# Hippogriff/prifit

Hardware: AMD Instinct MI355X
Metric: shapes/sec (fwd+bwd) B=24x2048 pts, PointNet++-MSG+ellipsoid fit (higher is better)
Workload: dtype f32; 1 GPU; configs[2]: PointNet++-MSG + mean-shift(10 it, <=25 clusters) + ellipsoid fit + convex loss, B=24x2048 per GPU, fwd+bwd+Adam; global_batch=24, points=2048, parallelism=dp1, cloud=blobs, embedding=clustered, backbone_grad_param=sa1.conv_blocks.0.0.weight, launch=eager

## Files before the change

include/prifit_hip.h:

```cpp
#ifndef PRIFIT_HIP_H
#define PRIFIT_HIP_H

#include <stdint.h>

#ifdef __cplusplus
extern "C" {
#endif

#define PRIFIT_OK 0
#define PRIFIT_EINVAL (-1)
#define PRIFIT_ELAUNCH (-2)

#define PRIFIT_ABI_VERSION 700
int prifit_version(const char **arch);


int prifit_fps(const float *xyz, int B, int N, int npoint, const int64_t *start_idx,
               int64_t *out_idx, float *new_xyz, void *stream);

int prifit_ball_query(const float *xyz, const float *new_xyz, int B, int N, int S, int R,
                      const float *radius2, const int *nsample, void *const *out, int idx64,
                      void *stream);

int prifit_three_nn(const float *xyz1, const float *xyz2, int B, int N, int S, int32_t *idx,
                    float *dist, float *weight, void *stream);

int prifit_square_distance(const float *src, const float *dst, int B, int S, int N, float *out,
                           void *stream);


int prifit_group_gather(const float *feat, const float *xyz, const float *new_xyz,
                        const int32_t *idx, int B, int N, int S, int K, int C, int order,
                        int ld_out, float *out, void *stream);

int prifit_group_scatter_add(const float *gout, int ld_gout, int col0, const int32_t *idx, int B,
                             int N, int S, int K, int C, float *dfeat, void *stream);
// ... 12 lines not shown

int prifit_three_interpolate_bwd(const float *gout, int ld_gout, int col0, const int32_t *idx,
                                 const float *weight, int B, int N, int S, int C, float *dpoints2,
                                 void *stream);
int prifit_fp_rows(const float *points2, const int32_t *idx, const float *weight, const float *points1, int B, int N, int S, int D2,
                   int D1, int kp, float *out, void *stream);


#define PRIFIT_GEMM_NT 0
#define PRIFIT_GEMM_NN 1
#define PRIFIT_GEMM_TN 2
#define PRIFIT_EPI_NONE 0
#define PRIFIT_EPI_CHORD 1
#define PRIFIT_EPI_MSKERNEL 2
#define PRIFIT_EPI_MSBWD 3

int prifit_gemm_f32(int layout, int M, int N, int K, const float *A, long long lda, long long strideA,
                    const float *B, long long ldb, long long strideB, float *C, long long ldc,
                    long long strideC, int batch, int splitk, const float *a_scale,
                    const float *a_shift, const float *b_scale, const float *b_shift,
                    const float *bias, long long bias_batch_stride, float *col_stats, int epilogue,
                    const float *epi_batch_scalar, const float *epi_aux, long long ld_aux,
                    long long stride_aux, const float *epi_row_add, float *a_rowsum, int accumulate, void *stream);

int prifit_chord_sym_f32(const float *A, long long lda, long long strideA, float *C, long long ldc, long long strideC,
                         int n, int K, int batch, unsigned long long *owner_key, void *stream);
int prifit_chord_sym_mask(const float *A, long long lda, long long strideA, const float *thr, uint32_t *mask, int n, int K, int batch,
                          unsigned long long *owner_key, void *stream);
int prifit_gram_sym_f32(const float *A, long long lda, long long strideA, float *C, long long ldc, long long strideC, int n, int K,
                        int batch, void *stream);

int prifit_gemm_pool_f32(int M, int N, int K, const float *A, long long lda, const float *W, long long ldb, float *Y,
                         long long ldc, const float *a_scale, const float *a_shift, const float *bias, float *col_stats,
                         float *cand, void *stream);
int prifit_gemm_pool_supported(int M, int N, int K);

int prifit_gemm_stream_f32(int layout, int M, int N, int K, const float *A, long long lda, const float *B,
                           long long ldb, float *C, long long ldc, const float *a_scale, const float *a_shift,
                           const float *bias, float *col_stats, void *stream);
int prifit_gemm_stream_supported(int layout, int M, int N, int K);
int prifit_gemm_stream_slabs(int M, int K);

int prifit_gemm_dual_nn_f32(int M, int N, int K1, int K2, const float *A1, const float *A2, long long lda,
                            long long strideA, const float *B1, const float *B2, long long ldb, long long strideB,
                            float *C, long long ldc, long long strideC, int batch, int splitk, int accumulate,
                            void *stream);
// ... 386 lines not shown
```

prifit_amd/_lib.py:

```python
import ctypes
import os
import re

import torch

_HERE = os.path.dirname(os.path.abspath(__file__))
LIB_PATH = os.environ.get("PRIFIT_LIB") or os.path.join(_HERE, "lib", "libprifit_hip.so")
HEADER_PATH = os.path.join(os.path.dirname(_HERE), "include", "prifit_hip.h")

_P = ctypes.c_void_p
_I = ctypes.c_int
_F = ctypes.c_float
_D = ctypes.c_double
_LL = ctypes.c_longlong

_dll = None


def declared_symbols(header_path=HEADER_PATH):
    return sorted(_declared(header_path))


def _declared(header_path=HEADER_PATH):
    with open(header_path) as f:
        text = f.read()
    return {name: ret for ret, name in re.findall(r"^\s*(int|long long)\s+(prifit_\w+)\s*\(", text, flags=re.M)}


def _ctype_of(param):
    p = param.strip()
    if p in ("void", ""):
        return None
    if "*" in p or "[" in p:
        return ctypes.c_void_p
    if re.search(r"\blong\s+long\b", p):
        return ctypes.c_ulonglong if "unsigned" in p else ctypes.c_longlong
    if re.search(r"\bdouble\b", p):
        return ctypes.c_double
    if re.search(r"\bfloat\b", p):
# ... 98 lines not shown
```

prifit_amd/csrc/gemm.hip:

```cpp
#include <stdlib.h>

#include <type_traits>

#include "common.h"

typedef float f32x16 __attribute__((ext_vector_type(16)));

enum { LAY_NT = 0, LAY_NN = 1, LAY_TN = 2 };
enum { EPI_NONE = 0, EPI_CHORD = 1, EPI_MSKERNEL = 2, EPI_MSBWD = 3, EPI_BNRED = 4 };

struct GemmArgs {
    const float *A, *B;
    float *C;
    int M, N, K;
    long long lda, ldb, ldc;
    long long sA, sB, sC;
    int batch, splitk;
    const float *a_scale, *a_shift;
    const float *b_scale, *b_shift;
    const float *bias;
    long long bias_stride;
    float *stats;
    int epi;
    const float *epi_batch_scalar;
    const float *aux;
    const float *row_add;
    float *a_rowsum;
    long long ldaux, sAux;
    const float *red_scale, *red_shift, *red_mean, *red_invstd;
    long long dA2, dB2;
    int kswitch;
    int accumulate;
    int vecA, vecB;
    int ntiles;
    float *cand;
};

#ifndef GEMM_W8
#define GEMM_W8 6
#endif
constexpr int BK = 32;
constexpr int PAD = 4;

__device__ __forceinline__ float4 ld4(const float *p) { return *reinterpret_cast<const float4 *>(p); }

template <int ROWS, bool KC, bool VEC, bool AFF, int NTH>
struct TileLoader {
    static constexpr int NV = ROWS * BK / 4 / NTH;
    static_assert(NV * NTH * 4 == ROWS * BK, "tile must divide evenly over the threads");
    float4 v[NV];
    const float *ptr[NV];
    int klo[NV];
    int c0[NV];
    unsigned okmask[NV];
    long long step;
    int K, R, cclamp;

    __device__ __forceinline__ void init(const float *__restrict__ base, long long ld, int r0, int R_, int K_)
    {
// ... 292 lines not shown
            fa[(gk + 1) & 1] = read_frag<RA, AKC>(As, arow, gk + 1, lh);
#pragma unroll
            for (int b = 0; b < TN; ++b)
                if (b < nbv) fb[(gk + 1) & 1][b] = read_frag<RB, BKC>(Bs, bcol + 32 * b, gk + 1, lh);
        }
        __builtin_amdgcn_sched_barrier(0);
        const float4 a = fa[gk & 1];
#pragma unroll
        for (int b = 0; b < TN; ++b) {
            if (b >= nbv) continue;
            const float4 w = fb[gk & 1][b];
            acc[b] = __builtin_amdgcn_mfma_f32_32x32x2f32(a.x, w.x, acc[b], 0, 0, 0);
            acc[b] = __builtin_amdgcn_mfma_f32_32x32x2f32(a.y, w.y, acc[b], 0, 0, 0);
            acc[b] = __builtin_amdgcn_mfma_f32_32x32x2f32(a.z, w.z, acc[b], 0, 0, 0);
            acc[b] = __builtin_amdgcn_mfma_f32_32x32x2f32(a.w, w.w, acc[b], 0, 0, 0);
        }
        __builtin_amdgcn_sched_barrier(0);
    }
}

template <bool C, class A, class B> struct pick { typedef A type; };
template <class A, class B> struct pick<false, A, B> { typedef B type; };

template <int BM, int BN, int WM, int WN, int LAY, bool VA, bool VB, bool FA, bool FB, bool EX = false>
__global__ __launch_bounds__((BM / WM) * (BN / WN) * 64, ((BM / WM) * (BN / WN) == 8 ? GEMM_W8 : 4)) void gemm_kernel(const GemmArgs g)
{
    constexpr int NTH = (BM / WM) * (BN / WN) * 64;
    constexpr bool A_KC = (LAY != LAY_TN);
    constexpr bool B_KC = (LAY == LAY_NT);
    constexpr int TM = WM / 32, TN = WN / 32;
    constexpr int WAVES_N = BN / WN;
    static_assert(NTH == 256 || NTH == 512, "4 or 8 waves per block");
    constexpr int SZA = A_KC ? BM * (BK + PAD) : BK * (BM + PAD);
    constexpr int SZB = B_KC ? BN * (BK + PAD) : BK * (BN + PAD);
    __shared__ __attribute__((aligned(16))) float lds[2 * (SZA + SZB)];

    const int tilesN = (g.N + BN - 1) / BN;
    const int nwg = gridDim.x;
    int L;
    {
        const int bid = blockIdx.x, xcd = bid & 7, pos = bid >> 3, q = nwg >> 3, r = nwg & 7;
        L = (xcd < r ? xcd * (q + 1) : r * (q + 1) + (xcd - r) * q) + pos;
    }
    const int tile_m = L / tilesN, tile_n = L - tile_m * tilesN;
    const int m0 = tile_m * BM, n0 = tile_n * BN;
    const int z = blockIdx.z / g.splitk, ks = blockIdx.z - z * g.splitk;

    const float *A = g.A + (long long)z * g.sA;
    const float *B = g.B + (long long)z * g.sB;
    float *C = g.C + (long long)z * g.sC;

    const int ktiles = (g.K + BK - 1) / BK;
    const int per = (ktiles + g.splitk - 1) / g.splitk;
    const int kt0 = ks * per, kt1 = min(ktiles, kt0 + per);

    const int wave = threadIdx.x >> 6, lane = threadIdx.x & 63;
    const int li = lane & 31, lh = lane >> 5;
    const int wm0 = (wave / WAVES_N) * WM, wn0 = (wave % WAVES_N) * WN;

    f32x16 acc[TM][TN];
#pragma unroll
    for (int a = 0; a < TM; ++a)
#pragma unroll
        for (int b = 0; b < TN; ++b)
#pragma unroll
            for (int r = 0; r < 16; ++r) acc[a][b][r] = 0.f;

    typename pick<EX, BufLoader<BM, A_KC, FA, NTH>, TileLoader<BM, A_KC, VA, FA, NTH>>::type la;
    typename pick<EX, BufLoader<BN, B_KC, FB, NTH>, TileLoader<BN, B_KC, VB, FB, NTH>>::type lb;
// ... 174 lines not shown
        }
    }
    if (g.stats) {
        __syncthreads();
        float *red = lds;
#pragma unroll
        for (int b = 0; b < TN; ++b) {
            float s = csum[b] + __shfl_xor(csum[b], 32, 64);
            float q = csq[b] + __shfl_xor(csq[b], 32, 64);
            if (lh == 0) {
                red[((wave / WAVES_N) * 2 + 0) * BN + wn0 + 32 * b + li] = s;
                red[((wave / WAVES_N) * 2 + 1) * BN + wn0 + 32 * b + li] = q;
            }
        }
        __syncthreads();
        for (int t = threadIdx.x; t < 2 * BN; t += NTH) {
            const int which = t / BN, c = t - which * BN;
            float s = 0.f;
#pragma unroll
            for (int w = 0; w < BM / WM; ++w) s += red[(w * 2 + which) * BN + c];
            if (n0 + c < g.N) g.stats[((long long)tile_m * 2 + which) * g.N + n0 + c] = s;
        }
    }
}

#ifdef PERS_STAMPS
__device__ unsigned long long g_pers_stamps[8 * 8 * 8];
__device__ int g_pers_ktail = 1;
#define PERS_STAMP(i)                                                                                       \
    do {                                                                                                     \
        if (st_slot >= 0 && st_tile < 8) {                                                                   \
            const unsigned long long t_ = __builtin_amdgcn_s_memtime();                                      \
            if (threadIdx.x == 0) g_pers_stamps[(st_slot * 8 + st_tile) * 8 + (i)] = t_;                    \
        }                                                                                                    \
    } while (0)
#else
#define PERS_STAMP(i) do { } while (0)
#endif

template <int LAY, bool FA, bool RED, bool PMAX = false>
__global__ __launch_bounds__(512) __attribute__((amdgpu_waves_per_eu(4, 4))) void gemm_pers_kernel(const GemmArgs g)
{
#ifdef PERS_STAMPS
    const int st_slot = (blockIdx.x % 61 == 0 && blockIdx.x / 61 < 8) ? (int)blockIdx.x / 61 : -1;
    int st_tile = 0;
#endif
// ... 531 lines not shown

static inline bool aligned16(const void *p) { return ((uintptr_t)p & 15) == 0; }

static inline bool small_tiles(int M, int N, int batch, int splitk)
{
    const long long wgs = (long long)((M + 127) / 128) * ((N + 127) / 128) * batch * splitk;
    return wgs < (splitk > 1 ? 160 : 520) && M > 64 && N > 32;
}

static int dispatch(GemmArgs &g, int layout, void *stream)
{
    const int M = g.M, N = g.N, K = g.K;
    const int extA = layout == LAY_TN ? M : K, extB = layout == LAY_NT ? K : N;
    g.vecA = aligned16(g.A) && (g.lda % 4 == 0) && (g.sA % 4 == 0) && (extA % 4 == 0);
    g.vecB = aligned16(g.B) && (g.ldb % 4 == 0) && (g.sB % 4 == 0) && (extB % 4 == 0);
    hipStream_t st = as_stream(stream);
    if (small_tiles(M, N, g.batch, g.splitk)) return launch_cfg<64, 64, 32, 32>(g, layout, st);
    if (N <= 32) return launch_cfg<128, 32, 32, 32>(g, layout, st);
    if (N <= 64) return launch_cfg<128, 64, 32, 64>(g, layout, st);
    if (N <= 96) return launch_cfg<128, 96, 32, 96>(g, layout, st);
    if (launch_persistent(g, layout, st)) return prifit_check_launch();
    if (layout == LAY_TN && launch_tnsk(g, st)) return prifit_check_launch();
    return launch_cfg<128, 128, 32, 64>(g, layout, st);
}

extern "C" {

#ifdef PERS_STAMPS
int prifit_debug_pers_ktail(int on)
{
    return hipMemcpyToSymbol(HIP_SYMBOL(g_pers_ktail), &on, sizeof(int)) == hipSuccess ? 0 : -1;
}
int prifit_debug_pers_stamps(unsigned long long *host, int n)
{
    return hipMemcpyFromSymbol(host, HIP_SYMBOL(g_pers_stamps), sizeof(unsigned long long) * (size_t)n) == hipSuccess ? 0 : -1;
}
#endif

int prifit_gemm_tile_m(int N)
{
    (void)N;
    return 128;
}

int prifit_gemm_stats_tile_m(int M, int N)
{
// ... 64 lines not shown
    }
    return dispatch(g, LAY_NN, stream);
}

int prifit_gemm_dgrad_bnred_f32(int M, int N, int K, const float *dY, long long lda, const float *W, long long ldb,
                                float *G, long long ldc, const float *Yprev, long long ldy, const float *scale,
                                const float *shift, const float *mean, const float *invstd, float *red_slab, void *stream)
{
    if (!dY || !W || !G || !Yprev || !scale || !shift || !mean || !invstd || !red_slab || M <= 0 || N <= 0 || K <= 0 ||
        lda < K || ldb < N || ldc < N || ldy < N)
        return PRIFIT_EINVAL;
    GemmArgs g;
    g.A = dY; g.B = W; g.C = G; g.M = M; g.N = N; g.K = K;
    g.lda = lda; g.ldb = ldb; g.ldc = ldc; g.sA = g.sB = g.sC = 0;
    g.batch = 1; g.splitk = 1;
    g.a_scale = g.a_shift = g.b_scale = g.b_shift = nullptr;
    g.bias = nullptr; g.bias_stride = 0; g.stats = red_slab; g.epi = EPI_BNRED; g.epi_batch_scalar = nullptr;
    g.accumulate = 0; g.aux = Yprev; g.ldaux = ldy; g.sAux = 0; g.row_add = nullptr; g.a_rowsum = nullptr;
    g.red_scale = scale; g.red_shift = shift; g.red_mean = mean; g.red_invstd = invstd;
    g.dA2 = g.dB2 = 0; g.kswitch = 0;
    return dispatch(g, LAY_NN, stream);
}

int prifit_chord_sym_f32(const float *A, long long lda, long long strideA, float *C, long long ldc, long long strideC,
                         int n, int K, int batch, unsigned long long *owner_key, void *stream)
{
    if (!A || !C || n <= 0 || (n % 128) || K <= 0 || (K % BK) || batch <= 0 || batch > 65535 || lda < K || ldc < n || (lda & 3) ||
        (ldc & 3) || (strideA & 3) || (strideC & 3) || ((uintptr_t)A & 15) || ((uintptr_t)C & 15) ||
        (long long)n * lda * 4 >= 0x7ff00000LL)
        return PRIFIT_EINVAL;
    const int T = n / 128;
    hipLaunchKernelGGL(chord_sym_kernel<0>, dim3((unsigned)(T * (T + 1) / 2 * batch)), dim3(512), 0, as_stream(stream), A, lda,
                       strideA, C, ldc, strideC, n, K, batch, owner_key, (const float *)nullptr, (unsigned *)nullptr);
    return prifit_check_launch();
}

int prifit_chord_sym_mask(const float *A, long long lda, long long strideA, const float *thr, uint32_t *mask, int n, int K, int batch,
                          unsigned long long *owner_key, void *stream)
{
    if (!A || !thr || !mask || n <= 0 || (n % 128) || K <= 0 || (K % BK) || batch <= 0 || batch > 65535 || lda < K || (lda & 3) ||
        (strideA & 3) || ((uintptr_t)A & 15) || (long long)n * lda * 4 >= 0x7ff00000LL)
        return PRIFIT_EINVAL;
    const int T = n / 128;
    hipLaunchKernelGGL(chord_sym_kernel<2>, dim3((unsigned)(T * (T + 1) / 2 * batch)), dim3(512), 0, as_stream(stream), A, lda,
                       strideA, (float *)nullptr, 0LL, 0LL, n, K, batch, owner_key, thr, mask);
    return prifit_check_launch();
// ... 53 lines not shown
```

prifit_amd/nn_ops.py:

```python
import collections
import ctypes
import os
import types

import torch

from . import profiler
from . import arena as zero_pool
from ._lib import call, cur_stream, dll, ptr, query

NT, NN, TN = 0, 1, 2
EPI_NONE, EPI_CHORD, EPI_MSKERNEL, EPI_MSBWD = 0, 1, 2, 3
_LL = ctypes.c_longlong
_F = ctypes.c_float
_D = ctypes.c_double


def _rows_per_slab():
    return query("prifit_reduce_rows_per_slab")


_STREAM = os.environ.get("PRIFIT_GEMM_STREAM", "1") != "0"
_FUSE_RED = os.environ.get("PRIFIT_FUSE_BN_REDUCE", "1") != "0"
_FUSE_POOL_FWD = os.environ.get("PRIFIT_FUSE_POOL_FWD", "1") != "0"
_FUSE_BN_APPLY = os.environ.get("PRIFIT_FUSE_BN_APPLY", "1") != "0"
_FUSE_POOL = os.environ.get("PRIFIT_FUSE_POOL_BWD", "1") != "0"
_FUSE_BWD = os.environ.get("PRIFIT_FUSE_DA_DW", "auto")

_FUSE_BWD_AUTO = {(96, 64), (64, 64), (128, 128)}


def _fuse_bwd_on(Cout, Kin, pooled):
    if _FUSE_BWD == "auto":
        return (Cout, Kin) in _FUSE_BWD_AUTO and not pooled
    return _FUSE_BWD not in ("0", "")
# ... 16 lines not shown
    call("prifit_slab_sum", ptr(part), part.shape[0], _LL(out.numel()), ptr(out), cur_stream())
    return out


def gemm_stats_slabs(M, N, K):
    if _stream_ok(NT, M, N, K):
        return query("prifit_gemm_stream_slabs", M, K)
    t = query("prifit_gemm_stats_tile_m", M, N)
    return (M + t - 1) // t


def gemm(layout, M, N, K, A, lda, B, ldb, C, ldc, batch=1, sA=0, sB=0, sC=0, splitk=1, a_affine=None,
         b_affine=None, bias=None, bias_stride=0, stats=None, epi=EPI_NONE, epi_scalar=None, aux=None, ld_aux=0, s_aux=0,
         row_add=None, a_rowsum=None, accumulate=None, tiled_stats=False):
    if accumulate is None:
        accumulate = splitk > 1
    if (not (tiled_stats and stats is not None) and _stream_ok(layout, M, N, K, batch, splitk, epi, b_affine, a_rowsum, accumulate, aux, row_add) and lda % 4 == 0 and
            A.data_ptr() % 16 == 0 and (layout == NN or (ldb % 4 == 0 and B.data_ptr() % 16 == 0))):
        with profiler.span(profiler.tag("gemm_stream_%s" % ("nt", "nn")[layout], M, N, K), 4.0 * (M * K + M * N + N * K)):
            call("prifit_gemm_stream_f32", layout, M, N, K, ptr(A), _LL(lda), ptr(B), _LL(ldb), ptr(C), _LL(ldc),
                 ptr(a_affine[0]) if a_affine else None, ptr(a_affine[1]) if a_affine else None, ptr(bias), ptr(stats),
                 cur_stream())
        return
    with profiler.span(profiler.tag("gemm_%s_bn%d" % (("nt", "nn", "tn")[layout], _bn_tile(N)), M, N, K, batch, splitk),
                       2.0 * M * N * K * batch):
        call("prifit_gemm_f32", layout, M, N, K, ptr(A), _LL(lda), _LL(sA), ptr(B), _LL(ldb), _LL(sB), ptr(C),
             _LL(ldc), _LL(sC), batch, splitk,
             ptr(a_affine[0]) if a_affine else None, ptr(a_affine[1]) if a_affine else None,
             ptr(b_affine[0]) if b_affine else None, ptr(b_affine[1]) if b_affine else None,
             ptr(bias), _LL(bias_stride), ptr(stats), epi, ptr(epi_scalar), ptr(aux), _LL(ld_aux), _LL(s_aux), ptr(row_add),
             ptr(a_rowsum), int(accumulate), cur_stream())


_SPLITK_WGS = 512


def _splitk_for(P, tiles):
    ktiles = (P + 31) // 32
    want = max(1, _SPLITK_WGS // max(1, tiles))
    return int(max(1, min(want, ktiles // 8 if ktiles >= 8 else 1, 4096)))


def _weight_grad(dY, P, Cout, Ain, Kin, a_affine, out=None):
    if _STREAM and query("prifit_gemm_stream_tn_supported", Cout, Kin, P):
        dW = out if out is not None else zero_pool.zeros(Cout, Kin, device=dY.device)
        ws = torch.empty(query("prifit_gemm_stream_tn_workspace", Cout, Kin, P), dtype=torch.float32, device=dY.device)
        with profiler.span(profiler.tag("gemm_stream_tn", Cout, Kin, P), 4.0 * P * (Cout + Kin)):
            call("prifit_gemm_stream_tn_f32", Cout, Kin, _LL(P), ptr(dY), _LL(dY.stride(0)), ptr(Ain), _LL(Ain.stride(0)),
                 ptr(dW), _LL(Kin), ptr(a_affine[0]) if a_affine else None, ptr(a_affine[1]) if a_affine else None,
                 ptr(ws), cur_stream())
        return dW
    tiles = ((Cout + 127) // 128) * ((Kin + 127) // 128)
    sk = _splitk_for(P, tiles)
    if out is not None:
        dW = out
    elif sk == 1:
        dW = torch.empty(Cout, Kin, dtype=torch.float32, device=dY.device)
    else:
        dW = zero_pool.zeros(Cout, Kin, device=dY.device)
    gemm(TN, Cout, Kin, P, dY, dY.stride(0), Ain, Ain.stride(0), dW, Kin, splitk=sk, b_affine=a_affine)
    return dW


def _forward_kernel(last, pool_K, aligned, has_affine, P, Cout, Kin):
    if last and pool_K and pool_K % 32 == 0 and _FUSE_POOL_FWD and aligned and has_affine:
        if _stream_ok(NT, P, Cout, Kin):
            return "stream_pool"
        if query("prifit_gemm_pool_supported", P, Cout, Kin):
            return "tiled_pool"
    return "gemm"


_Route = collections.namedtuple("_Route", "name kernel red")


def _backward_route(l, L, P, Cout, Kin, pool_K, training, mode, need_dW, need_dx, g_dense, g_contig, below_ld4, N0=0):
    pooled = l == L - 1 and bool(pool_K)

    def streams():
        return _stream_ok(NN, P, Kin, Cout) and bool(query("prifit_gemm_stream_tn_supported", Cout, Kin, P))

    if pooled and _FUSE_POOL and training and l > 0 and pool_K % 64 == 0 and Cout != 96 and need_dW and streams():
        if (_fuse_bwd_on(Cout, Kin, True) and _FUSE_RED and query("prifit_gemm_stream_bwd_supported", P, Cout, Kin, pool_K) and
# ... 126 lines not shown
            call("prifit_gather_linear_bwd_csr", ptr(G), ptr(Uq), ptr(Vq), ptr(ly.bias0), ptr(ly.scale), ptr(ly.shift),
                 ptr(ly.ca), ptr(ly.cb), ptr(ly.cd), ptr(fe.idx), ptr(offs), ptr(lst), ptr(own), Bq, Nq, Sq, Kq, Cout, ptr(dU),
                 ptr(dVc), ptr(wsd), cur_stream())
    else:
        dU = zero_pool.zeros(Bq, Nq, Cout, device=dev)
        dVc = zero_pool.zeros(Bq, Sq, Cout, device=dev)
        with profiler.span("gather_linear_bwd", 4.0 * (2.0 * P * Cout + P + (Bq * Nq + Bq * Sq) * Cout)):
            call("prifit_gather_linear_bwd_bn", ptr(G), ptr(ly.Y), ptr(ly.scale), ptr(ly.shift), ptr(ly.ca), ptr(ly.cb), ptr(ly.cd),
                 ptr(fe.idx), Bq, Nq, Sq, Kq, Cout, ptr(dU), ptr(dVc), cur_stream())
    return None, dU, None, dVc


def _route_plain(ly, route):
    P, Cout, Kin, G, W, Yp, dev = ly.P, ly.Cout, ly.Kin, ly.G, ly.W, ly.Yp, ly.dev
    dY = torch.empty(P, Cout, dtype=torch.float32, device=dev)
    if ly.pooled:
        call("prifit_pool_bwd_apply", ptr(G), _LL(G.stride(0)), ptr(ly.Y), _LL(Cout), ptr(ly.arg), ptr(ly.scale), ptr(ly.shift),
             ptr(ly.ca), ptr(ly.cb), ptr(ly.cd), P // ly.pool_K, ly.pool_K, Cout, 0, _F(0.0), ptr(dY), _LL(Cout), cur_stream())
    else:
        call("prifit_bn_relu_bwd_apply", ptr(G), _LL(G.stride(0)), ptr(ly.Y), _LL(Cout), ptr(ly.scale), ptr(ly.shift),
             ptr(ly.ca), ptr(ly.cb), ptr(ly.cd), P, Cout, 0, _F(0.0), ptr(dY), _LL(Cout), cur_stream())
    if route.name == "preact0":
        return dY, None, None, None
    dW = _weight_grad(dY, P, Cout, Yp, Kin, ly.aff_p, out=ly.dW) if ly.need_dW else None
    db = dY.sum(dim=0) if ly.want_db else None
    G_prev = None if route.kernel is None else torch.empty(P, Kin, dtype=torch.float32, device=dev)
    rslab = None
    if route.red:
        (sc1, sh1), (mu1, is1) = ly.aff_p, ly.stats_p
    if route.kernel == "gemm":
        gemm(NN, P, Kin, Cout, dY, Cout, W, Kin, G_prev, Kin)
    elif route.kernel == "stream":
        rslab = torch.empty(query("prifit_gemm_stream_slabs", P, Cout), 2, Kin, dtype=torch.float32, device=dev)
        with profiler.span(profiler.tag("gemm_stream_nn", P, Kin, Cout, 0), 4.0 * (P * Cout + 2 * P * Kin + Kin * Cout)):
            call("prifit_gemm_stream_dgrad_f32", P, Kin, Cout, ptr(dY), _LL(Cout), ptr(W), _LL(Kin), ptr(G_prev),
                 _LL(Kin), ptr(Yp), _LL(Yp.stride(0)), ptr(sc1), ptr(sh1), ptr(mu1), ptr(is1), ptr(rslab), cur_stream())
    elif route.kernel == "tiled":
        t = query("prifit_gemm_stats_tile_m", P, Kin)
        rslab = torch.empty((P + t - 1) // t, 2, Kin, dtype=torch.float32, device=dev)
        with profiler.span(profiler.tag("gemm_nn_bn%d" % _bn_tile(Kin), P, Kin, Cout, "red"), 2.0 * P * Kin * Cout):
            call("prifit_gemm_dgrad_bnred_f32", P, Kin, Cout, ptr(dY), _LL(Cout), ptr(W), _LL(Kin), ptr(G_prev),
                 _LL(Kin), ptr(Yp), _LL(Yp.stride(0)), ptr(sc1), ptr(sh1), ptr(mu1), ptr(is1), ptr(rslab), cur_stream())
    return G_prev, dW, rslab, db


_ROUTES = {"pool": _route_pool, "bn": _route_bn, "norows": _fused_bwd, "direct0": _route_direct0,
           "gather0": _route_gather0, "preact0": _route_plain, "plain": _route_plain}


def _eval_coeffs(gamma, beta, rmean, rvar, eps):
    invstd = torch.rsqrt(rvar + eps)
    mean = rmean.clone()
    scale = gamma * invstd
    return scale, beta - mean * scale, mean, invstd


FrontEnd = collections.namedtuple("FrontEnd", "mode slab idx B N S K D xyz new_xyz feat feat_first U Vc",
                                  defaults=(None,) * 12)


def _mlp_tensors(convs, bns, first_weight):
    ts = []
    for i, (conv, bn) in enumerate(zip(convs, bns)):
        w = first_weight if i == 0 else conv.weight.reshape(conv.weight.shape[0], -1)
# ... 354 lines not shown
    @staticmethod
    def forward(ctx, x, W, b):
        x = x.contiguous()
        W = W.contiguous()
        P, Kin = x.shape
        Cout = W.shape[0]
        sk = _few_rows_splitk(P, Cout, Kin)
        if sk > 1:
            Y = zero_pool.zeros(P, Cout, device=x.device)
            gemm(NT, P, Cout, Kin, x, Kin, W, Kin, Y, Cout, bias=b, splitk=sk)
        else:
            Y = torch.empty(P, Cout, dtype=torch.float32, device=x.device)
            gemm(NT, P, Cout, Kin, x, Kin, W, Kin, Y, Cout, bias=b)
        ctx.save_for_backward(x, W)
        return Y

    @staticmethod
    def backward(ctx, gy):
        x, W = ctx.saved_tensors
        gy = gy.contiguous()
        P, Kin = x.shape
        Cout = W.shape[0]
        dx = dW = db = None
        if ctx.needs_input_grad[0]:
            sk = _few_rows_splitk(P, Kin, Cout)
            if sk > 1:
                dx = zero_pool.zeros(P, Kin, device=x.device)
                gemm(NN, P, Kin, Cout, gy, Cout, W, Kin, dx, Kin, splitk=sk)
            else:
                dx = torch.empty(P, Kin, dtype=torch.float32, device=x.device)
                gemm(NN, P, Kin, Cout, gy, Cout, W, Kin, dx, Kin)
        if ctx.needs_input_grad[1]:
            dW = _weight_grad(gy, P, Cout, x, Kin, None)
        if ctx.needs_input_grad[2]:
            if Cout % 4 == 0 and gy.data_ptr() % 16 == 0:
                db = torch.empty(Cout, dtype=torch.float32, device=x.device)
                ws = torch.empty(query("prifit_col_sum_workspace", P, Cout), dtype=torch.float32, device=x.device)
                call("prifit_col_sum", ptr(gy), _LL(Cout), P, Cout, ptr(db), ptr(ws), cur_stream())
            else:
                db = gy.sum(dim=0)
        return dx, dW, db


class CrossEntropyFn(torch.autograd.Function):

    @staticmethod
    def forward(ctx, x, target):
        if x.stride(1) != 1:
            x = x.contiguous()
        target = target.contiguous()
        P, C = x.shape
        lse = torch.empty(P, dtype=torch.float32, device=x.device)
        ws = torch.empty(query("prifit_cross_entropy_workspace"), dtype=torch.float32, device=x.device)
        loss = torch.empty(2, dtype=torch.float32, device=x.device)
        call("prifit_cross_entropy_fwd", ptr(x), _LL(x.stride(0)), ptr(target), _LL(P), C, ptr(lse), ptr(ws), ptr(loss), cur_stream())
        ctx.save_for_backward(x, target, lse, loss)
# ... 112 lines not shown
```

Before: 1649 shapes/s.

## Batch independent backward GEMMs into one grouped kernel launch

Adds a grouped GEMM kernel that takes a table of up to four independent GEMM jobs and runs them in one launch, with each workgroup picking its job from cumulative tile counts. The backward passes of conv/BN layers and linear layers now defer the weight-grad and input-grad GEMMs and submit them together. The grouped path is only used when the jobs fit in one wave of resident workgroups and do not alias each other's outputs. The aim is to cut launch overhead and let small GEMMs fill the GPU at the same time, at the cost of forcing 64x64 tiles and extra host-side planning per call.

```diff
diff --git a/include/prifit_hip.h b/include/prifit_hip.h
--- a/include/prifit_hip.h
+++ b/include/prifit_hip.h
@@ -10,8 +10,9 @@
 #define PRIFIT_OK 0
 #define PRIFIT_EINVAL (-1)
 #define PRIFIT_ELAUNCH (-2)
-
-#define PRIFIT_ABI_VERSION 700
+#define PRIFIT_EUNSUPPORTED (-3)
+
+#define PRIFIT_ABI_VERSION 800
 int prifit_version(const char **arch);
 
 
@@ -70,6 +71,39 @@
                     const float *bias, long long bias_batch_stride, float *col_stats, int epilogue,
                     const float *epi_batch_scalar, const float *epi_aux, long long ld_aux,
                     long long stride_aux, const float *epi_row_add, float *a_rowsum, int accumulate, void *stream);
+
+typedef struct GemmArgs {
+    const float *A, *B;
+    float *C;
+    int M, N, K;
+    long long lda, ldb, ldc;
+    long long sA, sB, sC;
+    int batch, splitk;
+    const float *a_scale, *a_shift;
+    const float *b_scale, *b_shift;
+    const float *bias;
+    long long bias_stride;
+    float *stats;
+    int epi;
+    const float *epi_batch_scalar;
+    const float *aux;
+    const float *row_add;
+    float *a_rowsum;
+    long long ldaux, sAux;
+    const float *red_scale, *red_shift, *red_mean, *red_invstd;
+    long long dA2, dB2;
+    int kswitch;
+    int accumulate;
+    int vecA, vecB;
+    int ntiles;
+    float *cand;
+    int layout;
+} GemmArgs;
+#define PRIFIT_EPI_BNRED 4
+#define PRIFIT_GEMM_GROUP_MAX 4
+
+int prifit_gemm_group_supported(const GemmArgs *jobs, int n);
+int prifit_gemm_group_f32(const GemmArgs *jobs, int n, void *stream);
 
 int prifit_chord_sym_f32(const float *A, long long lda, long long strideA, float *C, long long ldc, long long strideC,
                          int n, int K, int batch, unsigned long long *owner_key, void *stream);
diff --git a/prifit_amd/_lib.py b/prifit_amd/_lib.py
--- a/prifit_amd/_lib.py
+++ b/prifit_amd/_lib.py
@@ -15,6 +15,18 @@
 _LL = ctypes.c_longlong
 
 _dll = None
+
+
+class GemmArgs(ctypes.Structure):
+    _fields_ = [("A", _P), ("B", _P), ("C", _P), ("M", _I), ("N", _I), ("K", _I), ("lda", _LL), ("ldb", _LL), ("ldc", _LL),
+                ("sA", _LL), ("sB", _LL), ("sC", _LL), ("batch", _I), ("splitk", _I), ("a_scale", _P), ("a_shift", _P),
+                ("b_scale", _P), ("b_shift", _P), ("bias", _P), ("bias_stride", _LL), ("stats", _P), ("epi", _I),
+                ("epi_batch_scalar", _P), ("aux", _P), ("row_add", _P), ("a_rowsum", _P), ("ldaux", _LL), ("sAux", _LL),
+                ("red_scale", _P), ("red_shift", _P), ("red_mean", _P), ("red_invstd", _P), ("dA2", _LL), ("dB2", _LL),
+                ("kswitch", _I), ("accumulate", _I), ("vecA", _I), ("vecB", _I), ("ntiles", _I), ("cand", _P), ("layout", _I)]
+
+
+GEMM_GROUP_MAX = 4
 
 
 def declared_symbols(header_path=HEADER_PATH):
diff --git a/prifit_amd/csrc/gemm.hip b/prifit_amd/csrc/gemm.hip
--- a/prifit_amd/csrc/gemm.hip
+++ b/prifit_amd/csrc/gemm.hip
@@ -9,32 +9,6 @@
 enum { LAY_NT = 0, LAY_NN = 1, LAY_TN = 2 };
 enum { EPI_NONE = 0, EPI_CHORD = 1, EPI_MSKERNEL = 2, EPI_MSBWD = 3, EPI_BNRED = 4 };
 
-struct GemmArgs {
-    const float *A, *B;
-    float *C;
-    int M, N, K;
-    long long lda, ldb, ldc;
-    long long sA, sB, sC;
-    int batch, splitk;
-    const float *a_scale, *a_shift;
-    const float *b_scale, *b_shift;
-    const float *bias;
-    long long bias_stride;
-    float *stats;
-    int epi;
-    const float *epi_batch_scalar;
-    const float *aux;
-    const float *row_add;
-    float *a_rowsum;
-    long long ldaux, sAux;
-    const float *red_scale, *red_shift, *red_mean, *red_invstd;
-    long long dA2, dB2;
-    int kswitch;
-    int accumulate;
-    int vecA, vecB;
-    int ntiles;
-    float *cand;
-};
 
 #ifndef GEMM_W8
 #define GEMM_W8 6
@@ -373,8 +347,22 @@
 template <bool C, class A, class B> struct pick { typedef A type; };
 template <class A, class B> struct pick<false, A, B> { typedef B type; };
 
-template <int BM, int BN, int WM, int WN, int LAY, bool VA, bool VB, bool FA, bool FB, bool EX = false>
-__global__ __launch_bounds__((BM / WM) * (BN / WN) * 64, ((BM / WM) * (BN / WN) == 8 ? GEMM_W8 : 4)) void gemm_kernel(const GemmArgs g)
+__device__ __forceinline__ void xcd_tile(int bid, int nwg, int tilesN, int &tile_m, int &tile_n)
+{
+    const int xcd = bid & 7, pos = bid >> 3, q = nwg >> 3, r = nwg & 7;
+    const int L = (xcd < r ? xcd * (q + 1) : r * (q + 1) + (xcd - r) * q) + pos;
+    tile_m = L / tilesN;
+    tile_n = L - tile_m * tilesN;
+}
+
+template <int BM, int BN, int LAY>
+constexpr int gemm_tile_lds()
+{
+    return 2 * ((LAY != LAY_TN ? BM * (BK + PAD) : BK * (BM + PAD)) + (LAY == LAY_NT ? BN * (BK + PAD) : BK * (BN + PAD)));
+}
+
+template <int BM, int BN, int WM, int WN, int LAY, bool VA, bool VB, bool FA, bool FB, bool EX, class GA>
+__device__ __forceinline__ void gemm_tile(const GA &g, const int tile_m, const int tile_n, const int bz, float *lds)
 {
     constexpr int NTH = (BM / WM) * (BN / WN) * 64;
     constexpr bool A_KC = (LAY != LAY_TN);
@@ -384,18 +372,10 @@
     static_assert(NTH == 256 || NTH == 512, "4 or 8 waves per block");
     constexpr int SZA = A_KC ? BM * (BK + PAD) : BK * (BM + PAD);
     constexpr int SZB = B_KC ? BN * (BK + PAD) : BK * (BN + PAD);
-    __shared__ __attribute__((aligned(16))) float lds[2 * (SZA + SZB)];
-
-    const int tilesN = (g.N + BN - 1) / BN;
-    const int nwg = gridDim.x;
-    int L;
-    {
-        const int bid = blockIdx.x, xcd = bid & 7, pos = bid >> 3, q = nwg >> 3, r = nwg & 7;
-        L = (xcd < r ? xcd * (q + 1) : r * (q + 1) + (xcd - r) * q) + pos;
-    }
-    const int tile_m = L / tilesN, tile_n = L - tile_m * tilesN;
+    static_assert(2 * (SZA + SZB) == gemm_tile_lds<BM, BN, LAY>(), "the caller's LDS block");
+
     const int m0 = tile_m * BM, n0 = tile_n * BN;
-    const int z = blockIdx.z / g.splitk, ks = blockIdx.z - z * g.splitk;
+    const int z = bz / g.splitk, ks = bz - z * g.splitk;
 
     const float *A = g.A + (long long)z * g.sA;
     const float *B = g.B + (long long)z * g.sB;
@@ -616,6 +596,15 @@
             if (n0 + c < g.N) g.stats[((long long)tile_m * 2 + which) * g.N + n0 + c] = s;
         }
     }
+}
+
+template <int BM, int BN, int WM, int WN, int LAY, bool VA, bool VB, bool FA, bool FB, bool EX = false>
+__global__ __launch_bounds__((BM / WM) * (BN / WN) * 64, ((BM / WM) * (BN / WN) == 8 ? GEMM_W8 : 4)) void gemm_kernel(const GemmArgs g)
+{
+    __shared__ __attribute__((aligned(16))) float lds[gemm_tile_lds<BM, BN, LAY>()];
+    int tile_m, tile_n;
+    xcd_tile(blockIdx.x, gridDim.x, (g.N + BN - 1) / BN, tile_m, tile_n);
+    gemm_tile<BM, BN, WM, WN, LAY, VA, VB, FA, FB, EX>(g, tile_m, tile_n, blockIdx.z, lds);
 }
 
 #ifdef PERS_STAMPS
@@ -1193,6 +1182,162 @@
     if (launch_persistent(g, layout, st)) return prifit_check_launch();
     if (layout == LAY_TN && launch_tnsk(g, st)) return prifit_check_launch();
     return launch_cfg<128, 128, 32, 64>(g, layout, st);
+}
+
+struct GemmGroup {
+    GemmArgs job[PRIFIT_GEMM_GROUP_MAX];
+    int cum[PRIFIT_GEMM_GROUP_MAX + 1];
+    int kind[PRIFIT_GEMM_GROUP_MAX];
+};
+static_assert(sizeof(GemmGroup) <= 4096 - 256, "the table travels by value: 4 KB of kernel arguments, some of it the runtime's");
+static_assert(PRIFIT_GEMM_GROUP_MAX == 4, "gemm_group_kernel compares against cum[1..3]");
+
+__global__ __launch_bounds__(256, 4) void gemm_group_kernel(const GemmGroup grp)
+{
+    __shared__ __attribute__((aligned(16))) float lds[gemm_tile_lds<64, 64, LAY_NT>()];
+    static_assert(gemm_tile_lds<64, 64, LAY_NN>() <= gemm_tile_lds<64, 64, LAY_NT>() &&
+                  gemm_tile_lds<64, 64, LAY_TN>() <= gemm_tile_lds<64, 64, LAY_NT>(), "one LDS block for every kind");
+    typedef const GemmGroup __attribute__((address_space(4))) KTab;
+    KTab &tab = *(KTab *)__builtin_amdgcn_kernarg_segment_ptr();
+    (void)grp;
+    const int bid = blockIdx.x;
+    const int j = (bid >= tab.cum[1]) + (bid >= tab.cum[2]) + (bid >= tab.cum[3]);
+    const auto &g = tab.job[j];
+    const int local = bid - tab.cum[j];
+    const int tilesN = (g.N + 63) / 64, nwg = ((g.M + 63) / 64) * tilesN;
+    const int bz = local / nwg;
+    int tile_m, tile_n;
+    xcd_tile(local - bz * nwg, nwg, tilesN, tile_m, tile_n);
+    switch (tab.kind[j]) {
+        case 0: gemm_tile<64, 64, 32, 32, LAY_NT, true, true, false, false, true>(g, tile_m, tile_n, bz, lds); break;
+        case 1: gemm_tile<64, 64, 32, 32, LAY_NT, true, true, true, false, true>(g, tile_m, tile_n, bz, lds); break;
+        case 2: gemm_tile<64, 64, 32, 32, LAY_NT, true, true, false, true, true>(g, tile_m, tile_n, bz, lds); break;
+        case 3: gemm_tile<64, 64, 32, 32, LAY_NN, true, true, false, false, true>(g, tile_m, tile_n, bz, lds); break;
+        case 4: gemm_tile<64, 64, 32, 32, LAY_NN, true, true, true, false, true>(g, tile_m, tile_n, bz, lds); break;
+        case 5: gemm_tile<64, 64, 32, 32, LAY_NN, true, true, false, true, true>(g, tile_m, tile_n, bz, lds); break;
+        case 6: gemm_tile<64, 64, 32, 32, LAY_TN, true, true, false, false, true>(g, tile_m, tile_n, bz, lds); break;
+        case 7: gemm_tile<64, 64, 32, 32, LAY_TN, true, true, true, false, true>(g, tile_m, tile_n, bz, lds); break;
+        case 8: gemm_tile<64, 64, 32, 32, LAY_TN, true, true, false, true, true>(g, tile_m, tile_n, bz, lds); break;
+        default: break;
+    }
+}
+
+struct ByteSpan { uintptr_t lo, hi; };
+static inline ByteSpan mat_span(const float *p, long long rows, long long cols, long long ld, long long batch, long long stride)
+{
+    if (!p) return ByteSpan{0, 0};
+    const uintptr_t lo = (uintptr_t)p;
+    return ByteSpan{lo, lo + 4 * (uintptr_t)((batch - 1) * stride + (rows - 1) * ld + cols)};
+}
+static inline bool overlaps(const ByteSpan &a, const ByteSpan &b) { return a.lo < b.hi && b.lo < a.hi; }
+
+static int job_spans(const GemmArgs &g, ByteSpan *out, ByteSpan *all)
+{
+    const int lay = g.layout;
+    const long long tilesM = (g.M + 63) / 64;
+    out[0] = mat_span(g.C, g.M, g.N, g.ldc, g.batch, g.sC);
+    out[1] = mat_span(g.stats, tilesM * 2, g.N, g.N, 1, 0);
+    int n = 0;
+    all[n++] = out[0];
+    all[n++] = out[1];
+    all[n++] = lay == LAY_TN ? mat_span(g.A, g.K, g.M, g.lda, g.batch, g.sA) : mat_span(g.A, g.M, g.K, g.lda, g.batch, g.sA);
+    all[n++] = lay == LAY_NT ? mat_span(g.B, g.N, g.K, g.ldb, g.batch, g.sB) : mat_span(g.B, g.K, g.N, g.ldb, g.batch, g.sB);
+    all[n++] = mat_span(g.aux, g.M, g.N, g.ldaux, 1, 0);
+    all[n++] = mat_span(g.bias, 1, g.N, 0, g.batch, g.bias_stride);
+    const long long ca = lay == LAY_TN ? g.M : g.K, cb = lay == LAY_NT ? g.K : g.N;
+    all[n++] = mat_span(g.a_scale, 1, ca, 0, 1, 0);
+    all[n++] = mat_span(g.a_shift, 1, ca, 0, 1, 0);
+    all[n++] = mat_span(g.b_scale, 1, cb, 0, 1, 0);
+    all[n++] = mat_span(g.b_shift, 1, cb, 0, 1, 0);
+    all[n++] = mat_span(g.red_scale, 1, g.N, 0, 1, 0);
+    all[n++] = mat_span(g.red_shift, 1, g.N, 0, 1, 0);
+    all[n++] = mat_span(g.red_mean, 1, g.N, 0, 1, 0);
+    all[n++] = mat_span(g.red_invstd, 1, g.N, 0, 1, 0);
+    return n;
+}
+
+static int group_kind(GemmArgs &g)
+{
+    const int lay = g.layout;
+    if (!g.A || !g.B || !g.C || g.M <= 0 || g.N <= 0 || g.K <= 0 || g.batch <= 0 || g.splitk <= 0 || lay < 0 || lay > 2 ||
+        (long long)g.batch * g.splitk > 65535 || (g.splitk > 1 && !g.accumulate) ||
+        ((g.a_scale == nullptr) != (g.a_shift == nullptr)) || ((g.b_scale == nullptr) != (g.b_shift == nullptr)) ||
+        (g.a_scale && g.b_scale) || g.a_rowsum || g.kswitch || g.row_add || g.epi_batch_scalar)
+        return -1;
+    if (g.epi == EPI_BNRED) {
+        if (lay != LAY_NN || g.batch != 1 || g.splitk != 1 || g.accumulate || !g.stats || !g.aux || !g.red_scale || !g.red_shift ||
+            !g.red_mean || !g.red_invstd || g.ldaux < g.N)
+            return -1;
+    } else if (g.epi != EPI_NONE) {
+        return -1;
+    }
+    if (g.stats && (g.batch != 1 || g.splitk != 1)) return -1;
+    if (!small_tiles(g.M, g.N, g.batch, g.splitk)) return -1;
+    const int extA = lay == LAY_TN ? g.M : g.K, extB = lay == LAY_NT ? g.K : g.N;
+    g.vecA = aligned16(g.A) && (g.lda % 4 == 0) && (g.sA % 4 == 0) && (extA % 4 == 0);
+    g.vecB = aligned16(g.B) && (g.ldb % 4 == 0) && (g.sB % 4 == 0) && (extB % 4 == 0);
+    const long long spanA = (lay == LAY_TN ? (long long)g.K * g.lda : (long long)g.M * g.lda) * 4;
+    const long long spanB = (lay == LAY_NT ? (long long)g.N * g.ldb : (long long)g.K * g.ldb) * 4;
+    if (!(g.vecA && g.vecB) || spanA >= 0x7ff00000LL || spanB >= 0x7ff00000LL) return -1;
+    return 3 * lay + (g.a_scale ? 1 : (g.b_scale ? 2 : 0));
+}
+
+static int group_slots()
+{
+    static const int slots = [] {
+        int dev = 0, per_cu = 0;
+        hipDeviceProp_t p;
+        if (hipGetDevice(&dev) != hipSuccess || hipGetDeviceProperties(&p, dev) != hipSuccess ||
+            hipOccupancyMaxActiveBlocksPerMultiprocessor(&per_cu, gemm_group_kernel, 256, 0) != hipSuccess)
+            return 0;
+        return per_cu * p.multiProcessorCount;
+    }();
+    return slots;
+}
+
+static bool group_plan(const GemmArgs *jobs, int n, GemmGroup &grp)
+{
+    if (!jobs || n < 1 || n > PRIFIT_GEMM_GROUP_MAX) return false;
+    int kind[PRIFIT_GEMM_GROUP_MAX], depth[PRIFIT_GEMM_GROUP_MAX], order[PRIFIT_GEMM_GROUP_MAX];
+    long long wgs[PRIFIT_GEMM_GROUP_MAX], total = 0;
+    GemmArgs tmp[PRIFIT_GEMM_GROUP_MAX];
+    for (int i = 0; i < n; ++i) {
+        tmp[i] = jobs[i];
+        if ((kind[i] = group_kind(tmp[i])) < 0) return false;
+        const GemmArgs &g = tmp[i];
+        wgs[i] = (long long)((g.M + 63) / 64) * ((g.N + 63) / 64) * g.batch * g.splitk;
+        total += wgs[i];
+        const int ktiles = (g.K + BK - 1) / BK;
+        depth[i] = (ktiles + g.splitk - 1) / g.splitk;
+    }
+    if (total > group_slots()) return false;
+    ByteSpan out[PRIFIT_GEMM_GROUP_MAX][2], all[PRIFIT_GEMM_GROUP_MAX][16];
+    int nall[PRIFIT_GEMM_GROUP_MAX];
+    for (int i = 0; i < n; ++i) nall[i] = job_spans(tmp[i], out[i], all[i]);
+    for (int i = 0; i < n; ++i)
+        for (int j = 0; j < n; ++j) {
+            if (i == j) continue;
+            for (int o = 0; o < 2; ++o)
+                for (int a = 0; a < nall[j]; ++a)
+                    if (overlaps(out[i][o], all[j][a])) return false;
+        }
+    for (int i = 0; i < n; ++i) order[i] = i;
+    for (int i = 1; i < n; ++i)
+        for (int k = i; k > 0 && depth[order[k]] > depth[order[k - 1]]; --k) { const int t = order[k]; order[k] = order[k - 1]; order[k - 1] = t; }
+    int at = 0;
+    for (int s = 0; s < PRIFIT_GEMM_GROUP_MAX; ++s) {
+        grp.cum[s] = at;
+        if (s < n) {
+            grp.job[s] = tmp[order[s]];
+            grp.kind[s] = kind[order[s]];
+            at += (int)wgs[order[s]];
+        } else {
+            grp.job[s] = tmp[order[0]];
+            grp.kind[s] = -1;
+        }
+    }
+    grp.cum[PRIFIT_GEMM_GROUP_MAX] = at;
+    return true;
 }
 
 extern "C" {
@@ -1303,6 +1448,21 @@
     return dispatch(g, LAY_NN, stream);
 }
 
+int prifit_gemm_group_supported(const GemmArgs *jobs, int n)
+{
+    GemmGroup grp;
+    return group_plan(jobs, n, grp) ? 1 : 0;
+}
+
+int prifit_gemm_group_f32(const GemmArgs *jobs, int n, void *stream)
+{
+    if (!jobs || n < 1) return PRIFIT_EINVAL;
+    GemmGroup grp;
+    if (!group_plan(jobs, n, grp)) return PRIFIT_EUNSUPPORTED;
+    hipLaunchKernelGGL(gemm_group_kernel, dim3((unsigned)grp.cum[PRIFIT_GEMM_GROUP_MAX]), dim3(256), 0, as_stream(stream), grp);
+    return prifit_check_launch();
+}
+
 int prifit_chord_sym_f32(const float *A, long long lda, long long strideA, float *C, long long ldc, long long strideC,
                          int n, int K, int batch, unsigned long long *owner_key, void *stream)
 {
diff --git a/prifit_amd/nn_ops.py b/prifit_amd/nn_ops.py
--- a/prifit_amd/nn_ops.py
+++ b/prifit_amd/nn_ops.py
@@ -7,10 +7,10 @@
 
 from . import profiler
 from . import arena as zero_pool
-from ._lib import call, cur_stream, dll, ptr, query
+from ._lib import GEMM_GROUP_MAX, GemmArgs, call, cur_stream, dll, ptr, query
 
 NT, NN, TN = 0, 1, 2
-EPI_NONE, EPI_CHORD, EPI_MSKERNEL, EPI_MSBWD = 0, 1, 2, 3
+EPI_NONE, EPI_CHORD, EPI_MSKERNEL, EPI_MSBWD, EPI_BNRED = 0, 1, 2, 3, 4
 _LL = ctypes.c_longlong
 _F = ctypes.c_float
 _D = ctypes.c_double
@@ -73,14 +73,93 @@
                  ptr(a_affine[0]) if a_affine else None, ptr(a_affine[1]) if a_affine else None, ptr(bias), ptr(stats),
                  cur_stream())
         return
+    _launch_job((_gemm_fields(layout, M, N, K, A, lda, B, ldb, C, ldc, batch, sA, sB, sC, splitk, a_affine, b_affine, bias, bias_stride,
+                              stats, epi, epi_scalar, aux, ld_aux, s_aux, row_add, a_rowsum, accumulate), None))
+
+
+def _gemm_fields(layout, M, N, K, A, lda, B, ldb, C, ldc, batch=1, sA=0, sB=0, sC=0, splitk=1, a_affine=None, b_affine=None,
+                 bias=None, bias_stride=0, stats=None, epi=EPI_NONE, epi_scalar=None, aux=None, ld_aux=0, s_aux=0, row_add=None,
+                 a_rowsum=None, accumulate=None):
+    if accumulate is None:
+        accumulate = splitk > 1
+    return (layout, M, N, K, ptr(A), lda, sA, ptr(B), ldb, sB, ptr(C), ldc, sC, batch, splitk,
+            ptr(a_affine[0]) if a_affine else None, ptr(a_affine[1]) if a_affine else None,
+            ptr(b_affine[0]) if b_affine else None, ptr(b_affine[1]) if b_affine else None,
+            ptr(bias), bias_stride, ptr(stats), epi, ptr(epi_scalar), ptr(aux), ld_aux, s_aux, ptr(row_add),
+            ptr(a_rowsum), int(accumulate))
+
+
+_FIELD_NAMES = ("layout", "M", "N", "K", "A", "lda", "sA", "B", "ldb", "sB", "C", "ldc", "sC", "batch", "splitk", "a_scale", "a_shift",
+                "b_scale", "b_shift", "bias", "bias_stride", "stats", "epi", "epi_batch_scalar", "aux", "ldaux", "sAux", "row_add",
+                "a_rowsum", "accumulate")
+_RED_NAMES = ("red_scale", "red_shift", "red_mean", "red_invstd")
+
+
+def gemm_job(layout, M, N, K, A, lda, B, ldb, C, ldc, red=None, **kw):
+    return (_gemm_fields(layout, M, N, K, A, lda, B, ldb, C, ldc, **kw), tuple(ptr(t) for t in red) if red else None)
+
+
+def _job_name(job):
+    f, red = job
+    return "%s%s" % (("nt", "nn", "tn")[f[0]], "red" if red else "")
+
+
+def _launch_job(job):
+    f, red = job
+    (layout, M, N, K, A, lda, sA, B, ldb, sB, C, ldc, sC, batch, splitk, a_scale, a_shift, b_scale, b_shift, bias, bias_stride, stats,
+     epi, epi_scalar, aux, ld_aux, s_aux, row_add, a_rowsum, accumulate) = f
+    if red:
+        with profiler.span(profiler.tag("gemm_nn_bn%d" % _bn_tile(N), M, N, K, "red"), 2.0 * M * N * K):
+            call("prifit_gemm_dgrad_bnred_f32", M, N, K, A, lda, B, ldb, C, ldc, aux, ld_aux, red[0], red[1], red[2], red[3], stats,
+                 cur_stream())
+        return
     with profiler.span(profiler.tag("gemm_%s_bn%d" % (("nt", "nn", "tn")[layout], _bn_tile(N)), M, N, K, batch, splitk),
                        2.0 * M * N * K * batch):
-        call("prifit_gemm_f32", layout, M, N, K, ptr(A), _LL(lda), _LL(sA), ptr(B), _LL(ldb), _LL(sB), ptr(C),
-             _LL(ldc), _LL(sC), batch, splitk,
-             ptr(a_affine[0]) if a_affine else None, ptr(a_affine[1]) if a_affine else None,
-             ptr(b_affine[0]) if b_affine else None, ptr(b_affine[1]) if b_affine else None,
-             ptr(bias), _LL(bias_stride), ptr(stats), epi, ptr(epi_scalar), ptr(aux), _LL(ld_aux), _LL(s_aux), ptr(row_add),
-             ptr(a_rowsum), int(accumulate), cur_stream())
+        call("prifit_gemm_f32", layout, M, N, K, A, lda, sA, B, ldb, sB, C, ldc, sC, batch, splitk, a_scale, a_shift, b_scale, b_shift,
+             bias, bias_stride, stats, epi, epi_scalar, aux, ld_aux, s_aux, row_add, a_rowsum, accumulate, cur_stream())
+
+
+_GROUP = os.environ.get("PRIFIT_GEMM_GROUP", "1") != "0"
+group_launches = 0
+
+
+def _job_args(job, out):
+    f, red = job
+    for name, v in zip(_FIELD_NAMES, f):
+        setattr(out, name, v)
+    if red:
+        out.epi = EPI_BNRED
+        for name, v in zip(_RED_NAMES, red):
+            setattr(out, name, v)
+
+
+def _group_table(jobs):
+    arr = (GemmArgs * len(jobs))()
+    for i, job in enumerate(jobs):
+        _job_args(job, arr[i])
+    return arr
+
+
+def group_supported(jobs):
+    return 0 < len(jobs) <= GEMM_GROUP_MAX and bool(dll().prifit_gemm_group_supported(_group_table(jobs), len(jobs)))
+
+
+def run_jobs(jobs):
+    global group_launches
+    n = len(jobs)
+    if _GROUP and 1 < n <= GEMM_GROUP_MAX:
+        arr = _group_table(jobs)
+        if dll().prifit_gemm_group_supported(arr, n):
+            name = "gemm_group_" + "+".join(_job_name(j) for j in jobs)
+            if profiler.SHAPES:
+                name += "[" + ";".join("x".join(str(d) for d in j[0][1:4] + j[0][13:15]) for j in jobs) + "]"
+            with profiler.span(name, sum(2.0 * j[0][1] * j[0][2] * j[0][3] * j[0][13] for j in jobs)):
+                call("prifit_gemm_group_f32", arr, n, cur_stream())
+            group_launches += 1
+            return True
+    for job in jobs:
+        _launch_job(job)
+    return False
 
 
 _SPLITK_WGS = 512
@@ -92,7 +171,7 @@
     return int(max(1, min(want, ktiles // 8 if ktiles >= 8 else 1, 4096)))
 
 
-def _weight_grad(dY, P, Cout, Ain, Kin, a_affine, out=None):
+def _weight_grad(dY, P, Cout, Ain, Kin, a_affine, out=None, defer=None):
     if _STREAM and query("prifit_gemm_stream_tn_supported", Cout, Kin, P):
         dW = out if out is not None else zero_pool.zeros(Cout, Kin, device=dY.device)
         ws = torch.empty(query("prifit_gemm_stream_tn_workspace", Cout, Kin, P), dtype=torch.float32, device=dY.device)
@@ -109,7 +188,10 @@
         dW = torch.empty(Cout, Kin, dtype=torch.float32, device=dY.device)
     else:
         dW = zero_pool.zeros(Cout, Kin, device=dY.device)
-    gemm(TN, Cout, Kin, P, dY, dY.stride(0), Ain, Ain.stride(0), dW, Kin, splitk=sk, b_affine=a_affine)
+    if defer is not None:
+        defer.append(gemm_job(TN, Cout, Kin, P, dY, dY.stride(0), Ain, Ain.stride(0), dW, Kin, splitk=sk, b_affine=a_affine))
+    else:
+        gemm(TN, Cout, Kin, P, dY, dY.stride(0), Ain, Ain.stride(0), dW, Kin, splitk=sk, b_affine=a_affine)
     return dW
 
 
@@ -282,24 +364,25 @@
              ptr(ly.ca), ptr(ly.cb), ptr(ly.cd), P, Cout, 0, _F(0.0), ptr(dY), _LL(Cout), cur_stream())
     if route.name == "preact0":
         return dY, None, None, None
-    dW = _weight_grad(dY, P, Cout, Yp, Kin, ly.aff_p, out=ly.dW) if ly.need_dW else None
+    jobs = []
+    dW = _weight_grad(dY, P, Cout, Yp, Kin, ly.aff_p, out=ly.dW, defer=jobs) if ly.need_dW else None
     db = dY.sum(dim=0) if ly.want_db else None
     G_prev = None if route.kernel is None else torch.empty(P, Kin, dtype=torch.float32, device=dev)
     rslab = None
     if route.red:
         (sc1, sh1), (mu1, is1) = ly.aff_p, ly.stats_p
     if route.kernel == "gemm":
-        gemm(NN, P, Kin, Cout, dY, Cout, W, Kin, G_prev, Kin)
-    elif route.kernel == "stream":
+        jobs.append(gemm_job(NN, P, Kin, Cout, dY, Cout, W, Kin, G_prev, Kin))
+    elif route.kernel == "tiled":
+        t = query("prifit_gemm_stats_tile_m", P, Kin)
+        rslab = torch.empty((P + t - 1) // t, 2, Kin, dtype=torch.float32, device=dev)
+        jobs.append(gemm_job(NN, P, Kin, Cout, dY, Cout, W, Kin, G_prev, Kin, red=(sc1, sh1, mu1, is1), aux=Yp, ld_aux=Yp.stride(0),
+                             stats=rslab))
+    run_jobs(jobs)
+    if route.kernel == "stream":
         rslab = torch.empty(query("prifit_gemm_stream_slabs", P, Cout), 2, Kin, dtype=torch.float32, device=dev)
         with profiler.span(profiler.tag("gemm_stream_nn", P, Kin, Cout, 0), 4.0 * (P * Cout + 2 * P * Kin + Kin * Cout)):
             call("prifit_gemm_stream_dgrad_f32", P, Kin, Cout, ptr(dY), _LL(Cout), ptr(W), _LL(Kin), ptr(G_prev),
-                 _LL(Kin), ptr(Yp), _LL(Yp.stride(0)), ptr(sc1), ptr(sh1), ptr(mu1), ptr(is1), ptr(rslab), cur_stream())
-    elif route.kernel == "tiled":
-        t = query("prifit_gemm_stats_tile_m", P, Kin)
-        rslab = torch.empty((P + t - 1) // t, 2, Kin, dtype=torch.float32, device=dev)
-        with profiler.span(profiler.tag("gemm_nn_bn%d" % _bn_tile(Kin), P, Kin, Cout, "red"), 2.0 * P * Kin * Cout):
-            call("prifit_gemm_dgrad_bnred_f32", P, Kin, Cout, ptr(dY), _LL(Cout), ptr(W), _LL(Kin), ptr(G_prev),
                  _LL(Kin), ptr(Yp), _LL(Yp.stride(0)), ptr(sc1), ptr(sh1), ptr(mu1), ptr(is1), ptr(rslab), cur_stream())
     return G_prev, dW, rslab, db
 
@@ -700,16 +783,20 @@
         P, Kin = x.shape
         Cout = W.shape[0]
         dx = dW = db = None
+        jobs = []
         if ctx.needs_input_grad[0]:
             sk = _few_rows_splitk(P, Kin, Cout)
             if sk > 1:
                 dx = zero_pool.zeros(P, Kin, device=x.device)
+            else:
+                dx = torch.empty(P, Kin, dtype=torch.float32, device=x.device)
+            if _stream_ok(NN, P, Kin, Cout, splitk=sk, accumulate=sk > 1):
                 gemm(NN, P, Kin, Cout, gy, Cout, W, Kin, dx, Kin, splitk=sk)
             else:
-                dx = torch.empty(P, Kin, dtype=torch.float32, device=x.device)
-                gemm(NN, P, Kin, Cout, gy, Cout, W, Kin, dx, Kin)
+                jobs.append(gemm_job(NN, P, Kin, Cout, gy, Cout, W, Kin, dx, Kin, splitk=sk))
         if ctx.needs_input_grad[1]:
-            dW = _weight_grad(gy, P, Cout, x, Kin, None)
+            dW = _weight_grad(gy, P, Cout, x, Kin, None, defer=jobs)
+        run_jobs(jobs)
         if ctx.needs_input_grad[2]:
             if Cout % 4 == 0 and gy.data_ptr() % 16 == 0:
                 db = torch.empty(Cout, dtype=torch.float32, device=x.device)
```

Result: no change. 1647 shapes/s (-0.1%).
